# kaiidams/Kokoro-Align

Measured on AMD Instinct MI355X. Metric: aligned audio-frames/sec (whole node), 50k x 5k lattice, higher is better.
Workload: dtype f32; 1 GPU; cfg2: T=50000 x V=64 log-probs, S=5000 phonemes (L=10001), beam_size=1000, max_move=4; batch of 8192 independent lattices per GPU per step, as 4 launches of 2048 on 4 streams; lattices_per_gpu=8192, parallelism=lattice-sharded x1, kernel_form=auto, backtrace=auto, streams_per_gpu=4

## Files before the change

kokoro-align_amd/csrc/ka_wave_backtrace.hpp:

```cpp
#pragma once
#include "ka_device.hpp"

namespace ka {

constexpr int kRcMinWaves = 8;

constexpr int kBtChunk = 16;
constexpr int kBtReach = 3 * 2 * kBtChunk;
constexpr int kBtBlocks = kBtChunk / 2;
constexpr int kBtRegs = kBtChunk * kBtBlocks / 64;
constexpr int kBtGroupsPerReg = 16 / kBtBlocks;
static_assert(16 * kBtBlocks >= kBtReach + 31, "window too narrow for the prefetch distance");

__device__ __forceinline__ int bt_window(int p_entry)
{
    const int lo = p_entry - kBtReach;
    return (lo > 0 ? lo : 0) >> 4;
}
__device__ __forceinline__ uint32_t bt_lane_offset(int w0, int lane)
{
    const int j = lane % kBtBlocks, fr = (lane / kBtBlocks) & 3, g = lane / (4 * kBtBlocks);
    return (uint32_t)g * 1024u + (uint32_t)((w0 + j) & 63) * 16u + (uint32_t)fr * 4u;
}
__device__ __forceinline__ void bt_load_guarded(uint32_t (&r)[kBtRegs], const char *chunk_base, int n, int w0, int lane)
{
    const int fr = (lane / kBtBlocks) & 3, g = lane / (4 * kBtBlocks);
    const uint32_t voff = bt_lane_offset(w0, lane);
#pragma unroll
    for (int v = 0; v < kBtRegs; ++v) {
        const int f = 4 * (v * kBtGroupsPerReg + g) + fr;
        r[v] = f < n ? *(gcu32_t)(chunk_base + (size_t)v * kBtGroupsPerReg * 1024 + voff) : 0u;
    }
}
__device__ __forceinline__ void bt_load_async(uint32_t (&r)[kBtRegs], const char *chunk_base , int w0, int lane)
{
    const uint32_t voff = bt_lane_offset(w0, lane);
#pragma unroll
    for (int v = 0; v < kBtRegs; ++v)
        asm volatile("global_load_dword %0, %1, %2" : "=&v"(r[v]) : "v"(voff), "s"(chunk_base + (size_t)v * kBtGroupsPerReg * 1024) : "memory");
}
template <int N>
__device__ __forceinline__ void bt_wait(uint32_t (&r)[2])
{
    asm volatile("s_waitcnt vmcnt(%2)" : "+v"(r[0]), "+v"(r[1]) : "i"(N) : "memory");
}
template <bool FULL>
__device__ __forceinline__ void bt_walk(const uint32_t (&r)[kBtRegs], int n, int w0, int &p, int &pathv)
{
    int q = p - 16 * w0;
    const int base = 16 * w0;
    uint32_t rr[kBtRegs];
#pragma unroll
    for (int i = 0; i < kBtRegs; ++i) rr[i] = blank_to_uniform(r[i]);
#pragma unroll
    for (int f = kBtChunk - 1; f >= 0; --f) {
        if (FULL || f < n) {
            const int grp = f >> 2;
            const int lane_base = ((grp % kBtGroupsPerReg) * 4 + (f & 3)) * kBtBlocks;
            const uint32_t w = (uint32_t)__builtin_amdgcn_readlane((int)rr[grp / kBtGroupsPerReg], (q >> 4) | lane_base);
            asm("v_writelane_b32 %0, %1, %2" : "+v"(pathv) : "s"(q), "i"(f));
            q -= bp_decode(w >> ((q * 2) & 31));
        }
    }
    pathv += base;
    p = q + base;
}

__global__ __launch_bounds__(64) void backtrace_w16_kernel(const Lattice *__restrict__ lats, const int32_t *meta, int only_flagged)
{
    const Lattice &d = lats[blockIdx.x];
    const int lane = threadIdx.x;
    if (only_flagged && !(__builtin_amdgcn_readfirstlane(meta[4 * (size_t)d.idx + 2]) & kFlagExact)) return;
    int p = __builtin_amdgcn_readfirstlane(meta[4 * (size_t)d.idx + 1]);
    if (p < 0) return;
    const char *bp = reinterpret_cast<const char *>(d.bp);
    gi32_t path = (gi32_t)d.path;
    const int T = __builtin_amdgcn_readfirstlane(d.T);
    uint32_t cur[kBtRegs], nxt[kBtRegs];
    int t0 = ((T - 1) / kBtChunk) * kBtChunk;
    int w = bt_window(p + 3 * kBtChunk);
    {
        const int n = T - t0;
        bt_load_guarded(cur, bp + (size_t)t0 * 256, n, w, lane);
        const int t1 = t0 > 0 ? t0 - kBtChunk : 0;
        const int wn = bt_window(p);
        bt_load_async(nxt, bp + (size_t)t1 * 256, wn, lane);
        int pathv = 0;
        bt_walk<false>(cur, n, w, p, pathv);
        if (lane < n) path[t0 + lane] = pathv;
        bt_wait<1>(nxt);
#pragma unroll
        for (int i = 0; i < kBtRegs; ++i) cur[i] = nxt[i];
        w = wn;
    }
    while (t0 > 0) {
        t0 -= kBtChunk;
        const int t1 = t0 > 0 ? t0 - kBtChunk : 0;
        const int wn = bt_window(p);
        bt_load_async(nxt, bp + (size_t)t1 * 256, wn, lane);
        int pathv = 0;
        bt_walk<true>(cur, kBtChunk, w, p, pathv);
        if (lane < kBtChunk) path[t0 + lane] = pathv;
        bt_wait<1>(nxt);
#pragma unroll
        for (int i = 0; i < kBtRegs; ++i) cur[i] = nxt[i];
        w = wn;
    }
}

__device__ __forceinline__ uint32_t rc_blank_to_uniform(uint32_t x)
{
    const uint32_t h = (x >> 3) & 0x11111111u, l = (x >> 2) & 0x11111111u;
    return (x & 0x33333333u) | ((h | l) << 3) | (h << 2);
}
__device__ __forceinline__ uint64_t lane_field(uint32_t count, uint32_t first)
{
    uint64_t m;
    asm("s_bfm_b64 %0, %1, %2" : "=s"(m) : "s"(count), "s"(first));
    return m;
}
#define KA_RC_E0_OUT "=&s"
#define KA_RC_E0_IN "s"
#define KA_RC_GATHER "ds_bpermute_b32 %[eln], %[lab4], %[rown]\n\tv_readfirstlane_b32 %[e0n], %[rown]\n\t"
#define KA_RC_HEAD                                                                        \
    KA_RC_GATHER                                                                          \
    "v_add_f32 %[t2], %[e0], %[sl]\n\t"                                                   \
    "v_add_f32_dpp %[t4], %[sl], %[el] wave_ror:1 row_mask:0xf bank_mask:0xf\n\t"         \
    "v_add_f32_dpp %[t5], %[sb], %[el] wave_ror:1 row_mask:0xf bank_mask:0xf\n\t"         \
    "v_add_f32 %[t0], %[e0], %[sb]\n\t"                                                   \
    "v_add_f32 %[t3], %[sb], %[el]\n\t"                                                   \
    "v_add_f32 %[t7], %[sl], %[el]\n\t"                                                   \
    "v_mov_b32_dpp %[t1], %[t2] wave_ror:1 row_mask:0xf bank_mask:0xf\n\t"                \
    "v_max_f32 %[t6], %[t7], %[t3]\n\t"
#define KA_RC_VETO "v_min_f32 %[t4], %[t4], %[veto]\n\t"
#define KA_RC_MAX                                                                         \
    "v_max3_f32 %[sl], %[t6], %[t4], %[t5]\n\t"                                           \
    "s_nop 0\n\t"                                                                         \
    "v_mov_b32_dpp %[t2], %[t1] wave_ror:1 row_mask:0xf bank_mask:0xf\n\t"                \
    "v_max3_f32 %[sb], %[t0], %[t1], %[t2]\n\t"
#define KA_RC_COMBINE                                                                     \
    "s_or_b64 %[sx], %[sa], %[sb2]\n\t"                                                   \
    "v_addc_co_u32 %[w], %[sy], %[w], %[w], %[sx]\n\t"                                    \
    "s_andn2_b64 %[sc], %[sc], %[sb2]\n\t"                                                \
    "s_or_b64 %[sc], %[sc], %[sa]\n\t"                                                    \
    "v_addc_co_u32 %[w], %[sy], %[w], %[w], %[sc]\n\t"
#define KA_RC_CODES                                                                       \
    "v_cmp_eq_f32 %[sa], %[t0], %[sb]\n\t"                                                \
    "v_addc_co_u32 %[w], %[sy], %[w], %[w], %[sa]\n\t"                                    \
    "v_cmp_eq_f32 %[sa], %[t1], %[sb]\n\t"                                                \
    "v_addc_co_u32 %[w], %[sy], %[w], %[w], %[sa]\n\t"                                    \
    "v_cmp_eq_f32 %[sa], %[t7], %[sl]\n\t"                                                \
    "v_cmp_eq_f32 %[sb2], %[t3], %[sl]\n\t"                                               \
    "v_cmp_eq_f32 %[sc], %[t4], %[sl]\n\t"                                                \
    KA_RC_COMBINE
#define KA_RC_BAND                                                                        \
    "s_bitcmp1_b32 %[open], 0\n\t"                                                        \
    "s_cbranch_scc1 .Lka_rc_open_%=\n\t"                                                  \
    "v_cndmask_b32 %[sb], %[ninf], %[sb], %[mb]\n\t"                                      \
    "v_cndmask_b32 %[sl], %[ninf], %[sl], %[ml]\n"                                        \
    ".Lka_rc_open_%=:\n\t"                                                                \
    "s_waitcnt lgkmcnt(0)"
#define KA_RC_OUTS                                                                                                              \
    [sb] "+v"(sb), [sl] "+v"(sl), [w] "+v"(word), [eln] "=&v"(el_next), [e0n] KA_RC_E0_OUT(e0_next), [t0] "=&v"(t0), [t1] "=&v"(t1),   \
    [t2] "=&v"(t2), [t3] "=&v"(t3), [t4] "=&v"(t4), [t5] "=&v"(t5), [t6] "=&v"(t6), [t7] "=&v"(t7), [sa] "=&s"(sa),             \
    [sb2] "=&s"(sb2), [sc] "=&s"(sc), [sx] "=&s"(sx), [sy] "=&s"(sy)
#define KA_RC_INS                                                                                                               \
    [e0] KA_RC_E0_IN(e0), [el] "v"(el), [rown] "v"(row_next), [lab4] "v"(lab4), [zero] "v"(zero), [open] "s"(open), [mb] "s"(mask_b),   \
    [ml] "s"(mask_l), [ninf] "v"(NINF)
template <bool ZL>
__device__ __forceinline__ void rc_frame4(float &sb, float &sl, uint32_t &word, float e0, float el, float &e0_next, float &el_next,
                                          float row_next, int lab4, int zero, float veto, uint32_t open, uint64_t mask_b,
                                          uint64_t mask_l, float NINF)
{
    float t0, t1, t2, t3, t4, t5, t6, t7;
    uint64_t sa, sb2, sc, sx, sy;
    if constexpr (ZL)
        asm volatile(KA_RC_HEAD KA_RC_VETO KA_RC_MAX KA_RC_CODES KA_RC_BAND : KA_RC_OUTS : KA_RC_INS, [veto] "v"(veto) : "memory", "scc");
    else
        asm volatile(KA_RC_HEAD KA_RC_MAX KA_RC_CODES KA_RC_BAND : KA_RC_OUTS : KA_RC_INS : "memory", "scc");
}
#undef KA_RC_HEAD
#undef KA_RC_GATHER
#undef KA_RC_E0_OUT
#undef KA_RC_E0_IN
#undef KA_RC_VETO
#undef KA_RC_MAX
#undef KA_RC_CODES
#undef KA_RC_COMBINE
#undef KA_RC_BAND
#undef KA_RC_OUTS
#undef KA_RC_INS
constexpr int kRcLanes = 62;

template <bool FULL>
__device__ __forceinline__ void rc_walk_out(const uint32_t (&codes)[kCkFrames / 8], const float (&rows)[kCkFrames], int lab4, int n,
                                            int &qq, int &pathv, int &labv, float &scv)
{
#pragma unroll
    for (int f = kCkFrames - 1; f >= 0; --f) {
        if (FULL || f < n) {
            const int j = qq >> 1;
            const int sh = 4 * (7 - (f & 7)) + ((qq & 1) ? 0 : 2);
            const uint32_t w = (uint32_t)__builtin_amdgcn_readlane((int)codes[f >> 3], j) >> sh;
            const int col = (qq & 1) ? __builtin_amdgcn_readlane(lab4, j) >> 2 : 0;
            const int sc = __builtin_amdgcn_readlane(__builtin_bit_cast(int, rows[f]), col);
            asm("v_writelane_b32 %0, %1, %2" : "+v"(pathv) : "s"(qq), "i"(f));
            asm("v_writelane_b32 %0, %1, %2" : "+v"(labv) : "s"(col), "i"(f));
            asm("v_writelane_b32 %0, %1, %2" : "+v"(scv) : "s"(sc), "i"(f));
            qq -= bp_decode(w);
        }
    }
}

template <int M, bool ZL, bool PAR>
__device__ __forceinline__ void backtrace_rc_body(const Lattice *__restrict__ lats, const int32_t *meta, int n_lats)
{
    const int which = PAR ? __builtin_amdgcn_readfirstlane(lattice_of_chunk(lats, n_lats, (int64_t)blockIdx.x)) : (int)blockIdx.x;
    const Lattice &d = lats[which];
    const int lane = threadIdx.x;
    if (!PAR && __builtin_amdgcn_readfirstlane(d.par)) return;
    const int32_t *mt = meta + 4 * (size_t)d.idx;
    const int flags = __builtin_amdgcn_readfirstlane(mt[2]);
    if (flags & (kFlagExact | kFlagDeclined)) return;
    if (((flags & kFlagZeroLabel) != 0) != ZL) return;
    if (__builtin_amdgcn_readfirstlane(mt[0]) != kStatusOk) return;
    int p = __builtin_amdgcn_readfirstlane(mt[1]);
    if (p < 0) return;
    const uint32_t T = (uint32_t)__builtin_amdgcn_readfirstlane(d.T);
    const uint32_t L = (uint32_t)__builtin_amdgcn_readfirstlane(d.L);
    const uint32_t B = (uint32_t)__builtin_amdgcn_readfirstlane(d.beam);
    const uint32_t halfB = B >> 1;
    const uint32_t dq = L / T, dr = L % T;
    const float NINF = ninf();
    const char *lp = reinterpret_cast<const char *>(d.lp);
    const size_t ldb = (size_t)d.ld * 4;
    const uint32_t col_off = (lane < d.V ? (uint32_t)lane : 0u) * 4u;
    gci32_t labx = (gci32_t)d.labx;
    const char *ck = reinterpret_cast<const char *>(d.bp);
    const uint32_t ck_mask = (uint32_t)__builtin_amdgcn_readfirstlane((int)d.ck_mask);
    const size_t ck_pitch = (size_t)(uint32_t)__builtin_amdgcn_readfirstlane(d.ck_pitch);
    gi32_t path = (gi32_t)d.path;
    gi32_t lab_out = (gi32_t)d.lab_out;
    gf32_t sc_out = (gf32_t)d.sc_out;

    uint32_t t0 = ((T - 1) / kCkFrames) * kCkFrames;
    if constexpr (PAR) {
        const uint32_t c = (uint32_t)((int64_t)blockIdx.x - d.chunk0);
        t0 = c * kCkFrames;
        p = __builtin_amdgcn_readfirstlane(d.entry[c]);
    }
    const auto uni = [](uint64_t v) { return (uint32_t)__builtin_amdgcn_readfirstlane((int)(uint32_t)v); };
    uint32_t q0 = uni(((uint64_t)L * t0) / T), r0 = uni(((uint64_t)L * t0) % T);
    const uint32_t D32 = uni(((uint64_t)L * kCkFrames) / T), R32 = uni(((uint64_t)L * kCkFrames) % T);
    const float inv_T = 1.0f / (float)T;

    for (;;) {
        const int n = (int)(T - t0 < (uint32_t)kCkFrames ? T - t0 : (uint32_t)kCkFrames);
        const int wlo = __builtin_amdgcn_readfirstlane((p > 96 ? p - 96 : 0) & ~1);
        const int pb = wlo + 2 * lane;
        int lab4;
        asm volatile("global_load_dword %0, %1, %2" : "=v"(lab4) : "v"((uint32_t)lane * 4u), "s"(labx + (wlo >> 1)) : "memory");
        f32x2 ckv = {NINF, NINF};
        if (t0 != 0) {
            const uint32_t off = ((uint32_t)pb & ck_mask) * 4u;
            asm volatile("global_load_dwordx2 %0, %1, %2" : "=v"(ckv) : "v"(off), "s"(ck + ((size_t)(t0 / kCkFrames) - 1) * ck_pitch) : "memory");
        }
        float rows[kCkFrames];
        {
            const char *rp = lp + (size_t)t0 * ldb;
            if (n == kCkFrames) {
#pragma unroll
                for (int f = 0; f < kCkFrames; ++f) {
                    rows[f] = row_load(col_off, rp);
                    rp += ldb;
                }
            } else {
#pragma unroll
                for (int f = 0; f < kCkFrames; ++f) {
                    rows[f] = row_load(col_off, rp);
                    rp += (f + 1 < n) ? ldb : 0;
                }
            }
        }
        asm volatile("s_waitcnt vmcnt(%2)" : "+v"(lab4), "+v"(ckv) : "i"(kCkFrames) : "memory");
        const float veto = lab4 == 0 ? NINF : __builtin_inff();
        float sb, sl;
        if (t0 == 0) {
            sb = pb == 0 ? 0.0f : NINF;
            sl = NINF;
        } else {
            const uint32_t qm = r0 >= dr ? q0 - dq : q0 - dq - 1;
            const int32_t dl = (int32_t)qm - (int32_t)halfB;
            const uint32_t lo1 = (uint32_t)(dl > 0 ? dl : 0);
            const uint32_t hi1 = (L - lo1 < B) ? L : lo1 + B;
            sb = ((uint32_t)pb >= lo1 && (uint32_t)pb < hi1 && lane < kRcLanes) ? ckv.x : NINF;
            sl = ((uint32_t)pb + 1 >= lo1 && (uint32_t)pb + 1 < hi1 && lane < kRcLanes) ? ckv.y : NINF;
        }
        uint32_t codes[kCkFrames / 8] = {};
        const auto div_T = [&](uint32_t x) {
            uint32_t qe = (uint32_t)((float)x * inv_T);
            qe -= (qe * T > x) ? 1u : 0u;
            qe += (x - qe * T >= T) ? 1u : 0u;
            return qe;
        };
        const uint32_t qnum = r0 + (uint32_t)lane * dr;
        const uint32_t qa = q0 + (uint32_t)lane * dq + div_T(qnum);
        uint64_t mask_b = 0, mask_l = 0;
        const auto band_masks = [&](int f) {
            const uint32_t q = (uint32_t)__builtin_amdgcn_readlane((int)qa, f);
            const int32_t dl = (int32_t)q - (int32_t)halfB;
            const int32_t lo = dl > 0 ? dl : 0;
            const int32_t hi = (L - (uint32_t)lo < B) ? (int32_t)L : lo + (int32_t)B;
            int32_t x = lo - wlo, y = hi - wlo;
            x = x < 0 ? 0 : x;
            y = y < 0 ? 0 : y;
            asm("" : "+s"(x), "+s"(y));
            x = x > 2 * kRcLanes ? 2 * kRcLanes : x;
            y = y > 2 * kRcLanes ? 2 * kRcLanes : y;
            const uint32_t xb = (uint32_t)(x + 1) >> 1, yb = (uint32_t)(y + 1) >> 1, xl = (uint32_t)x >> 1, yl = (uint32_t)y >> 1;
            mask_b = lane_field(yb - xb, xb);
            mask_l = lane_field(yl - xl, xl);
        };
        if constexpr (M == 4) {
            bool open = false;
            if (t0 != 0 && n == kCkFrames) {
                const uint32_t q_last = (uint32_t)__builtin_amdgcn_readlane((int)qa, kCkFrames - 1);
                const int32_t dl_last = (int32_t)q_last - (int32_t)halfB;
                const uint32_t qm = r0 >= dr ? q0 - dq : q0 - dq - 1;
                const int32_t dl = (int32_t)qm - (int32_t)halfB;
                const uint32_t lo1 = (uint32_t)(dl > 0 ? dl : 0);
                const uint32_t hi1 = (L - lo1 < B) ? L : lo1 + B;
                open = wlo > 0 && dl_last <= wlo && (uint32_t)p < hi1;
            }
            const int zero = 0;
            float e0c, elc, e0n, eln;
            row_wait_n(rows[0], kCkFrames - 1);
            asm volatile("ds_bpermute_b32 %0, %2, %4\n\t"
                         "v_readfirstlane_b32 %1, %4\n\t"
                         "s_waitcnt lgkmcnt(0)"
                         : "=&v"(elc), "=&s"(e0c) : "v"(lab4), "v"(zero), "v"(rows[0]) : "memory");
            uint32_t moves = 0;
            const uint32_t open_bit = (uint32_t)__builtin_amdgcn_readfirstlane(open ? 1 : 0);
            if (open_bit) {
                sb = ckv.x;
                sl = ckv.y;
            } else {
                const uint32_t qb = q0 + (uint32_t)(lane + 1) * dq + div_T(qnum + dr);
                moves = (uint32_t)__builtin_amdgcn_ballot_w64(qa != qb) << 1 | 1u;
            }
            asm volatile("s_nop 1" : "+v"(sb), "+v"(sl));
#pragma unroll
            for (int f = 0; f < kCkFrames; ++f) {
                if ((moves >> f) & 1u) band_masks(f);
                if (f + 1 < kCkFrames) row_wait_n(rows[f + 1], kCkFrames - 2 - f);
                rc_frame4<ZL>(sb, sl, codes[f >> 3], e0c, elc, e0n, eln, rows[f + 1 < kCkFrames ? f + 1 : f], lab4, zero, veto,
                              open_bit, mask_b, mask_l, NINF);
                e0c = e0n;
                elc = eln;
            }
        } else {
            const uint32_t qb = q0 + (uint32_t)(lane + 1) * dq + div_T(qnum + dr);
            const uint32_t moves = (uint32_t)__builtin_amdgcn_ballot_w64(qa != qb);
#pragma unroll
            for (int f = 0; f < kCkFrames; ++f) {
                if (f == 0 || ((moves >> (f > 0 ? f - 1 : 0)) & 1u)) band_masks(f);
                row_wait_n(rows[f], kCkFrames - 1 - f);
                const float el = bperm(lab4, rows[f]);
                const float e0 = first_lane(rows[f]);
                const float L1 = wave_ror1(sl);
                const float B1 = wave_ror1(sb);
                const float L2 = wave_ror1(L1);
                uint32_t &word = codes[f >> 3];
                if ((f & 7) == 0) word = 0;
                float mb, ml;
                cell_blank<M>(sb, L1, L2, e0, mb, word);
                cell_label<M, ZL>(sl, sb, L1, B1, el, veto, ml, word);
                sb = select_by_mask(NINF, mb, mask_b);
                sl = select_by_mask(NINF, ml, mask_l);
            }
        }
#pragma unroll
        for (int g = 0; g < kCkFrames / 8; ++g) codes[g] = rc_blank_to_uniform(codes[g]);
        int pathv = 0;
        int qq = p - wlo;
        int labv = 0;
        float scv = 0.0f;
        if (n == kCkFrames)
            rc_walk_out<true>(codes, rows, lab4, n, qq, pathv, labv, scv);
        else
            rc_walk_out<false>(codes, rows, lab4, n, qq, pathv, labv, scv);
        if (lane < n) {
            path[t0 + lane] = pathv + wlo;
            lab_out[t0 + lane] = labv;
            sc_out[t0 + lane] = scv;
        }
        p = qq + wlo;
        if (PAR || t0 == 0) break;
        t0 -= kCkFrames;
        q0 -= D32;
        if (r0 < R32) { r0 += T; q0 -= 1; }
        r0 -= R32;
    }
}

template <int M, bool ZL, bool PAR>
__global__ __launch_bounds__(64, kRcMinWaves) void backtrace_rc_kernel(const Lattice *__restrict__ lats, const int32_t *meta, int n_lats)
{
    backtrace_rc_body<M, ZL, PAR>(lats, meta, n_lats);
}
template <int M>
__global__ __launch_bounds__(64, kRcMinWaves) void backtrace_rc_chunks_kernel(const Lattice *__restrict__ lats, const int32_t *meta, int n_lats)
{
    const Lattice &d = lats[__builtin_amdgcn_readfirstlane(lattice_of_chunk(lats, n_lats, (int64_t)blockIdx.x))];
    const int flags = __builtin_amdgcn_readfirstlane(meta[4 * (size_t)d.idx + 2]);
    if (flags & kFlagZeroLabel)
        backtrace_rc_body<M, true, true>(lats, meta, n_lats);
    else
        backtrace_rc_body<M, false, true>(lats, meta, n_lats);
}

__global__ __launch_bounds__(256) void gather_outputs_kernel(const Lattice *__restrict__ lats, const int32_t *meta, int only_flagged)
{
    const Lattice &d = lats[blockIdx.y];
    if (meta[4 * (size_t)d.idx + 1] < 0) return;
    if (only_flagged && !(meta[4 * (size_t)d.idx + 2] & kFlagExact)) return;
    const int T = d.T;
    gci32_t path = (gci32_t)d.path;
    gci32_t labx = (gci32_t)d.labx;
    gcf32_t lp = (gcf32_t)d.lp;
    const size_t ld = (size_t)d.ld;
    for (int base = blockIdx.x * 1024; base < T; base += gridDim.x * 1024) {
        int t[4], pp[4], lab[4];
        float sc[4];
#pragma unroll
        for (int i = 0; i < 4; ++i) {
            t[i] = base + i * 256 + threadIdx.x;
            pp[i] = t[i] < T ? path[t[i]] : 0;
        }
#pragma unroll
        for (int i = 0; i < 4; ++i) lab[i] = (pp[i] & 1) ? (labx[pp[i] >> 1] >> 2) : 0;
#pragma unroll
        for (int i = 0; i < 4; ++i) sc[i] = t[i] < T ? lp[(size_t)t[i] * ld + lab[i]] : 0.0f;
#pragma unroll
        for (int i = 0; i < 4; ++i) {
            if (t[i] < T) {
                ((gi32_t)d.lab_out)[t[i]] = lab[i];
                ((gf32_t)d.sc_out)[t[i]] = sc[i];
            }
        }
    }
}


__global__ __launch_bounds__(64) void backtrace_generic_kernel(const Lattice *__restrict__ lats, const int32_t *meta)
{
    const Lattice &d = lats[blockIdx.x];
    const int lane = threadIdx.x;
    int64_t p = meta[4 * (size_t)d.idx + 1];
    if (p < 0) return;
    const int64_t T = d.T, L = d.L, B = d.beam, W = d.W;
    const uint8_t *bp = reinterpret_cast<const uint8_t *>(d.bp);
    if (lane == 0) {
        for (int64_t t = T - 1; t >= 0; --t) {
            int64_t lo = (L * t) / T - B / 2;
            lo = lo < 0 ? 0 : lo;
            d.path[t] = (int32_t)p;
            p -= bp[(size_t)t * (size_t)W + (size_t)(p - lo)];
        }
    }
}


}
```

Measured before the change: 6.808 billion frames/s.

## Walk backtrace codes two frames per readlane and vectorise label/score outputs

Backpointer codes are repacked with DPP and byte-permute so that one readlane fetches the codes for two consecutive frames. The serial backward walk then takes two steps per cross-lane read, and the label and score lookups move off the serial chain into a post-pass using ds_bpermute and packed columns. The blank-to-uniform conversion is also rewritten with v_bfi. This shortens the dependent scalar chain per frame but adds repacking work and more intricate bit indexing.

Result: no change. 6.852 billion frames/s, median of 6 (+0.7%).

```diff
diff --git a/kokoro-align_amd/csrc/ka_wave_backtrace.hpp b/kokoro-align_amd/csrc/ka_wave_backtrace.hpp
--- a/kokoro-align_amd/csrc/ka_wave_backtrace.hpp
+++ b/kokoro-align_amd/csrc/ka_wave_backtrace.hpp
@@ -110,8 +110,11 @@
 
 __device__ __forceinline__ uint32_t rc_blank_to_uniform(uint32_t x)
 {
-    const uint32_t h = (x >> 3) & 0x11111111u, l = (x >> 2) & 0x11111111u;
-    return (x & 0x33333333u) | ((h | l) << 3) | (h << 2);
+    const uint32_t t = x | (x << 1), s = x >> 1;
+    uint32_t u, r;
+    asm("v_bfi_b32 %0, %1, %2, %3" : "=v"(u) : "s"(0x88888888u), "v"(t), "v"(x));
+    asm("v_bfi_b32 %0, %1, %2, %3" : "=v"(r) : "s"(0x44444444u), "v"(s), "v"(u));
+    return r;
 }
 __device__ __forceinline__ uint64_t lane_field(uint32_t count, uint32_t first)
 {
@@ -192,23 +195,51 @@
 #undef KA_RC_INS
 constexpr int kRcLanes = 62;
 
+__device__ __forceinline__ void rc_pair_codes(uint32_t c, uint32_t &out_lo, uint32_t &out_hi)
+{
+    const uint32_t below = (uint32_t)__builtin_amdgcn_mov_dpp((int)c, 0x13C, 0xF, 0xF, false);
+    const uint32_t e = ((c >> 4) & 0x0F0F0F0Fu) | (below & 0xF0F0F0F0u);
+    const uint32_t d = (uint32_t)__builtin_amdgcn_mov_dpp((int)e, 0x13C, 0xF, 0xF, false);
+    out_lo = __builtin_amdgcn_perm(d, c, 0x05010400u);
+    out_hi = __builtin_amdgcn_perm(d, c, 0x07030602u);
+}
 template <bool FULL>
-__device__ __forceinline__ void rc_walk_out(const uint32_t (&codes)[kCkFrames / 8], const float (&rows)[kCkFrames], int lab4, int n,
-                                            int &qq, int &pathv, int &labv, float &scv)
-{
-#pragma unroll
-    for (int f = kCkFrames - 1; f >= 0; --f) {
-        if (FULL || f < n) {
-            const int j = qq >> 1;
-            const int sh = 4 * (7 - (f & 7)) + ((qq & 1) ? 0 : 2);
-            const uint32_t w = (uint32_t)__builtin_amdgcn_readlane((int)codes[f >> 3], j) >> sh;
-            const int col = (qq & 1) ? __builtin_amdgcn_readlane(lab4, j) >> 2 : 0;
-            const int sc = __builtin_amdgcn_readlane(__builtin_bit_cast(int, rows[f]), col);
-            asm("v_writelane_b32 %0, %1, %2" : "+v"(pathv) : "s"(qq), "i"(f));
-            asm("v_writelane_b32 %0, %1, %2" : "+v"(labv) : "s"(col), "i"(f));
-            asm("v_writelane_b32 %0, %1, %2" : "+v"(scv) : "s"(sc), "i"(f));
-            qq -= bp_decode(w);
-        }
+__device__ __forceinline__ void rc_walk(const uint32_t (&pairs)[kCkFrames / 4], int n, int &qq, int &pathv)
+{
+#pragma unroll
+    for (int k = kCkFrames / 2 - 1; k >= 0; --k) {
+        const int b = 3 - (k & 3);
+        const int reg = 2 * (k >> 2) + (b >> 1), sh = 16 * (b & 1);
+        if (!FULL && k == 0) qq = __builtin_amdgcn_readfirstlane(qq);
+        const uint32_t w = (uint32_t)__builtin_amdgcn_readlane((int)pairs[reg], qq >> 1);
+        const int s1 = sh + ((qq & 1) ? 0 : 2), s2 = s1 + 4;
+        if (FULL || 2 * k + 1 < n) {
+            asm("v_writelane_b32 %0, %1, %2" : "+v"(pathv) : "s"(qq), "i"(2 * k + 1));
+            const int m1 = bp_decode(w >> s1);
+            qq -= m1;
+            asm("v_writelane_b32 %0, %1, %2" : "+v"(pathv) : "s"(qq), "i"(2 * k));
+            int s3;
+            asm("s_lshl1_add_u32 %0, %1, %2" : "=s"(s3) : "s"(m1), "s"(s2) : "scc");
+            qq -= bp_decode(w >> s3);
+        } else if (k == 0 || 2 * k < n) {
+            asm("v_writelane_b32 %0, %1, %2" : "+v"(pathv) : "s"(qq), "i"(2 * k));
+            qq -= bp_decode(w >> s2);
+        }
+    }
+}
+__device__ __forceinline__ void rc_outputs(const float (&rows)[kCkFrames], int lab4, int pathv, int &labv, float &scv)
+{
+    const int cell = __builtin_amdgcn_ds_bpermute((pathv >> 1) << 2, lab4);
+    labv = (pathv & 1) ? cell >> 2 : 0;
+    int pk = labv | (__builtin_amdgcn_mov_dpp(labv, 0xF5, 0xF, 0xF, false) << 8);
+    pk |= __builtin_amdgcn_mov_dpp(pk, 0xAA, 0xF, 0xF, false) << 16;
+    int cols[kCkFrames / 4];
+#pragma unroll
+    for (int g = 0; g < kCkFrames / 4; ++g) cols[g] = __builtin_amdgcn_readlane(pk, 4 * g);
+#pragma unroll
+    for (int f = 0; f < kCkFrames; ++f) {
+        const int sc = __builtin_amdgcn_readlane(__builtin_bit_cast(int, rows[f]), (cols[f >> 2] >> (8 * (f & 3))) & 0xFF);
+        asm("v_writelane_b32 %0, %1, %2" : "+v"(scv) : "s"(sc), "i"(f));
     }
 }
 
@@ -379,16 +410,18 @@
                 sl = select_by_mask(NINF, ml, mask_l);
             }
         }
-#pragma unroll
-        for (int g = 0; g < kCkFrames / 8; ++g) codes[g] = rc_blank_to_uniform(codes[g]);
+        uint32_t pairs[kCkFrames / 4];
+#pragma unroll
+        for (int g = 0; g < kCkFrames / 8; ++g) rc_pair_codes(rc_blank_to_uniform(codes[g]), pairs[2 * g], pairs[2 * g + 1]);
         int pathv = 0;
         int qq = p - wlo;
-        int labv = 0;
+        if (n == kCkFrames)
+            rc_walk<true>(pairs, n, qq, pathv);
+        else
+            rc_walk<false>(pairs, n, qq, pathv);
+        int labv;
         float scv = 0.0f;
-        if (n == kCkFrames)
-            rc_walk_out<true>(codes, rows, lab4, n, qq, pathv, labv, scv);
-        else
-            rc_walk_out<false>(codes, rows, lab4, n, qq, pathv, labv, scv);
+        rc_outputs(rows, lab4, pathv, labv, scv);
         if (lane < n) {
             path[t0 + lane] = pathv + wlo;
             lab_out[t0 + lane] = labv;
```
